# algbio/SBWT

Hardware: AMD Instinct MI355X
Metric: k-mers/sec (whole node), plain-matrix k=30 streaming search (higher is better)
Workload: dtype u64

## Files before the change

### sbwt_amd/csrc/sbwt_device.h

```cpp
#pragma once
#include <stdint.h>

#ifndef SBWT_MEGA_SHIFT
#define SBWT_MEGA_SHIFT 31
#endif
static_assert(SBWT_MEGA_SHIFT >= 7 && SBWT_MEGA_SHIFT <= 31, "a mega block holds 2 .. 2^25 whole 64-column blocks, and its relative counts fit 32 bits");
#define SBWT_GROUP_BASES 32

#ifndef SBWT_FUSED_SORT_DEFAULT
#define SBWT_FUSED_SORT_DEFAULT 3632
#endif
struct SbwtIndexView {
    const uint4 *blocks;
    const longlong2 *ptab;
    const unsigned long long *mega;
    long long n_nodes;
    long long n_pos;
    long long C[4];
    int k;
    int p_dev;
    int n_mega;
    int has_ssup;
    int probe_len;
    const uint4 *stab;
    int p_sparse;
    unsigned n_sb;
    const unsigned *col, *pos;
    const uint4 *pq;
    int has_safe;
    const uint4 *stab2;
    unsigned n_sb2;
    const uint4 *pfil;
    int p_filter, log2f;
    const uint4 *trans;
    unsigned n_tslots;
    int stab_pos;
    int debug;
    int out32 = 0;
    int big = 0;
    int fused_sort = 0;
    int force_mega;
};

struct SbwtBlobHeader {
    uint64_t magic;
    int64_t n_nodes, n_kmers, k, p_file, p_dev;
    int64_t C[4];
    int64_t n_blocks, n_mega;
    int64_t off_blocks, off_ptab, off_ftab, off_mega, blob_bytes;
    int32_t has_ssup;
    int32_t rank_only;
    int32_t ssup_derived;
    int32_t p_sparse;
    int64_t off_stab;
    int32_t big_layout;
    int32_t has_path;
    int64_t off_col, off_pos, off_pq, off_trans;
    int32_t stab_pos;
    int32_t p_filter;
    int64_t off_pfil;
    int32_t log2f;
    int32_t has_safe;
    int32_t force_mega;
    int64_t n_tslots;
    int64_t n_sb;
    int64_t n_pos;
    int64_t n_trans;
    int64_t n_paths;
    int64_t n_branch;
    int64_t image_level;
    int64_t row_ones[4];
    int32_t log2b2_unused;
    int64_t n_sb2;
    int64_t off_stab2;
    int64_t path_lookahead;
};
#define SBWT_BLOB_MAGIC 0x3355504754574253ull

#define SBWT_SP_EMPTY (1ull << 63)
#define SBWT_SP_OVERFLOW (1ull << 62)
#define SBWT_SP_UNIQ 0x80000000u
#define SBWT_SP_MAX_DEPTH 31
#define SBWT_SP_HASH 0x9E3779B97F4A7C15ull
static __host__ __device__ inline unsigned long long sp2_hash(unsigned origin, unsigned long long key2) {
    unsigned long long h = (key2 ^ ((unsigned long long)origin << 17)) * SBWT_SP_HASH;
    h ^= h >> 31;
    return (h + origin) * 0xD6E8FEB86659FD93ull;
}
#define SBWT_SP2_USED 0x80000000u
#define SBWT_SP2_OVERFLOW 0x80000000u
static __host__ __device__ inline unsigned long long sbwt_pf_hash(unsigned long long key) { return key * SBWT_SP_HASH; }
static __host__ __device__ inline unsigned sbwt_pf_bits(unsigned long long h) { return (unsigned)(h >> 24) ^ (unsigned)(h >> 41); }

struct SbwtWorkHeader {
    unsigned long long ticket;
    int status;
    int rg_sample;
    unsigned long long n_stream;
    unsigned long long n_search;
    unsigned long long n_lf;
    unsigned long long n_tab_hit;
    unsigned long long n_ext;
    unsigned long long n_bridge;
    unsigned long long u_bad;
    long long u_read0, u_len, u_out0, u_stride;
    unsigned long long n_deferred;
    unsigned long long ticket2;
    unsigned long long n_pieces;
    unsigned long long pad[15];
    unsigned long long rg_long;
    unsigned long long n_ftick;
    unsigned long long ftick_over;
    unsigned long long pad2[5];
    unsigned long long hint;
};
#define SBWT_WS_CLEAR_BYTES (sizeof(SbwtWorkHeader) - 8)

#define SBWT_PIECE 1024
struct SbwtPieceTab {
    uint4 *pairs = nullptr;
    uint4 *outs = nullptr;
    long long cap = 0;
    int piece = SBWT_PIECE;
};
static_assert(sizeof(SbwtWorkHeader) == 320, "workspace header is 320 bytes");
struct SbwtTickTab {
    uint4 *tick = nullptr;
    unsigned *tick_read = nullptr;
    unsigned *defer_bits = nullptr;
    long long cap = 0;
};
#define SBWT_HINT_MAGIC 0x5B377A00u
#define SBWT_HINT_RATIO 12
#define SBWT_HINT_CALLS 2

void sbwt_launch_encode(const char *d_bases, long long total_bases, uint4 *d_packed, SbwtWorkHeader *ws,
                        hipStream_t stream);
void sbwt_launch_search(const SbwtIndexView &ix, const uint4 *d_packed, const long long *d_read_off,
                        const long long *d_out_off, long long *d_out, long long n_reads, SbwtWorkHeader *ws,
                        int streaming, hipStream_t stream, int variant, long long total_groups, void *d_sort_scratch,
                        long long sort_scratch_bytes, int sort_key_bits, SbwtPieceTab pt);
void sbwt_launch_search_fused(const SbwtIndexView &ix, const char *d_bases, long long total_bases, uint4 *d_packed,
                              const long long *d_read_off, const long long *d_out_off, long long *d_out, long long n_reads,
                              SbwtWorkHeader *ws, int streaming, hipStream_t stream, unsigned *d_defer,
                              hipEvent_t ev_begin, hipEvent_t ev_end, SbwtPieceTab pt, int ragged_ok, SbwtTickTab tt = SbwtTickTab());
void sbwt_launch_encode_chained(const char *d_bases, long long total_bases, uint4 *d_packed, SbwtWorkHeader *ws,
                                const unsigned *d_defer, const long long *d_read_off, int k, hipStream_t stream);
void sbwt_launch_search_chained(const SbwtIndexView &ix, const uint4 *d_packed, const long long *d_read_off,
                                const long long *d_out_off, long long *d_out, long long n_reads, SbwtWorkHeader *ws,
                                int streaming, hipStream_t stream, const unsigned *d_defer, SbwtPieceTab pt);
void sbwt_launch_piece_bounds_tt(const uint4 *d_packed, const long long *d_read_off, const long long *d_out_off, int k,
                                 SbwtWorkHeader *ws, SbwtPieceTab pt, int behind_fused, hipStream_t stream, const unsigned *defer_bits);
void sbwt_launch_piece_bounds(const uint4 *d_packed, const long long *d_read_off, const long long *d_out_off, int k,
                              SbwtWorkHeader *ws, SbwtPieceTab pt, int behind_fused, hipStream_t stream);
long long sbwt_sort_scratch_bytes(long long n_reads, int key_bits);
const unsigned *sbwt_launch_sort_reads(const SbwtIndexView &ix, const uint4 *d_packed, const long long *d_read_off,
                                       long long n_reads, const SbwtWorkHeader *ws, void *d_scratch, long long scratch_bytes,
                                       int key_bits, hipStream_t stream);
void sbwt_launch_rank(const SbwtIndexView &ix, const long long *d_pos, const char *d_sym, long long n,
                      long long *d_out, hipStream_t stream);
void sbwt_launch_precalc(const SbwtIndexView &ix, int p, longlong2 *d_table, hipStream_t stream);
void sbwt_launch_update_interval(const SbwtIndexView &ix, const char *d_bases, const long long *d_off, long long n,
                                 long long *d_first, long long *d_second, hipStream_t stream);
void sbwt_launch_forward(const SbwtIndexView &ix, const long long *d_node, const char *d_sym, long long n,
                         long long *d_out, hipStream_t stream);
void sbwt_launch_partial_search(const SbwtIndexView &ix, const char *d_bases, const long long *d_off, long long n,
                                long long *d_first, long long *d_second, long long *d_matched, hipStream_t stream);
void sbwt_launch_get_kmer(const SbwtIndexView &ix, const long long *d_colex, long long n, char *d_out,
                          hipStream_t stream);
void sbwt_launch_select(const SbwtIndexView &ix, const long long *d_j, const char *d_sym, long long n,
                        const long long row_ones[4], long long *d_out, hipStream_t stream);
long long sbwt_format_scratch_bytes(long long n_reads);
void sbwt_launch_format(const long long *d_vals, const long long *d_out_off, long long n_reads, char *d_text,
                        long long *d_line_off, void *d_scratch, hipStream_t stream);
long long sbwt_blocks_scratch_bytes(long long n_nodes);
int sbwt_blocks_count(const unsigned long long *d_bits, long long n_nodes, void *d_scratch, long long totals[5], hipStream_t st);
void sbwt_blocks_fill(const unsigned long long *d_bits, const unsigned long long *d_ssup, long long n_nodes, void *d_scratch,
                      const long long C[4], int use_mega, int n_mega, uint4 *d_blocks, unsigned long long *d_mega, hipStream_t st);
long long sbwt_derive_scratch_bytes(long long n_nodes);
void sbwt_launch_derive_marks(const SbwtIndexView &ix, uint4 *d_blocks, void *d_scratch, hipStream_t stream);
long long sbwt_sparse_scratch_bytes(long long n_nodes);
long long sbwt_path_scratch_bytes(long long n_nodes);
long long sbwt_path_quads(long long n_nodes);
long long sbwt_count_paths(const SbwtIndexView &ix, hipStream_t stream);
void sbwt_launch_path_safe(const SbwtIndexView &ix, uint4 *d_pq, int rule, void *d_hlab, unsigned char *d_alt_safe,
                           hipStream_t stream);
long long sbwt_path_safe_scratch_bytes(long long n_pos, int k);
long long sbwt_launch_path_oth(const SbwtIndexView &ix, uint4 *d_pq, long long *n_branch, hipStream_t stream, int count_only = 0);
void sbwt_launch_trans_insert(const SbwtIndexView &ix, uint4 *d_trans, long long n_slots, const unsigned char *d_alt_safe,
                              hipStream_t stream);
int sbwt_launch_build_path(const SbwtIndexView &ix, unsigned *d_col, unsigned *d_pos, uint4 *d_pq, long long pos_cap,
                           long long *n_pos, int stitch, int min_copy, void *d_scratch, int lookahead, hipStream_t stream);
int sbwt_launch_build_sparse(const SbwtIndexView &ix, int p_dense, int p_sparse, long long n_buckets, uint4 *d_table,
                             void *d_scratch, const unsigned *d_pos, int p_filter, int log2f, uint4 *d_filter,
                             long long n_entries2, uint4 *d_table2, hipStream_t stream);

struct SbwtBuildState {
    int k = 0, rc = 0, ssup = 0;
    int key_bytes = 8;
    long long n_text = 0, nk = 0, ng = 0, n_nopred = 0;
    void *km = nullptr;
    unsigned *edges = nullptr;
    void *nopred_keys = nullptr;
};
int sbwt_build_phase_a(const char *h_text, long long n_text, int k, int rc, SbwtBuildState *S, hipStream_t st);
int sbwt_build_from_keys(void *d_km, long long nk, int k, SbwtBuildState *S, hipStream_t st);
int sbwt_build_copy_nopred(const SbwtBuildState *S, void *h_keys);
int sbwt_build_phase_b(SbwtBuildState *S, const void *h_ddata, const unsigned *h_dedges, long long nd, int ssup,
                       unsigned long long *h_rows, hipStream_t st);
void sbwt_build_release(SbwtBuildState *S);
```

### sbwt_amd/csrc/sbwt_search_fused.hip

```cpp
#include "sbwt_kernels_common.h"

#define F_IDLE 0
#define F_INIT 2
#define F_STEP 3
#define F_DEAD 4
#define F_EXT 7
#define F_TRANS 8
#define F_POS 9
#define F_BRIDGE 10
#define F_CMP 11
#define F_PLAN 12
#define FE_NONE 0
#define FE_EMIT1 1
#define FE_FAIL 2
#define FE_END 3
#define FE_PRES 4
#define FE_ANCH 5
#ifndef FZ_ANCHORS
#define FZ_ANCHORS 3
#endif
#ifndef FZ_ALIGNS
#define FZ_ALIGNS 7
#endif
#define CF_S1 1u
#define CF_A1 2u
#define CF_B1 4u
#define CF_S2 8u
#define CF_A2 16u
#define CF_B2 32u
#define CF_ONP 64u
#define CF_ALIGNED 128u
#define CF_ANCH 256u
#define CF_SEED 512u
#define CA_GOON 0
#define CA_DONE 1
#define CA_CERT 2
#define CA_TRANS 3
#define CA_ABSENT 4
#define CA_LOST 5
#define CF_MISS 1024u
#define CF_MISS_MASK 3072u
#define CF_WIN31 8192u
#define CF_SEED2 16384u
#define CF_NOCERT 4096u
#define CF_FORCE (1u << 30)
#define CF_ANC_LEFT(f) (((f) >> 16) & 3u)
#define CF_CMP_LEFT(f) (((f) >> 18) & 7u)
#define CF_ANC_TRIED(f) ((int)(((f) >> 21) & 511u) - 1)
#define CF_SET_TRIED(f, a) ((f) = ((f) & ~(511u << 21)) | ((((unsigned)((a) + 1)) & 511u) << 21))
#define CF_BUDGETS (((unsigned)FZ_ANCHORS << 16) | ((unsigned)FZ_ALIGNS << 18))
#define CF_M1 (CF_S1 | CF_A1 | CF_B1)
#define CF_M2 (CF_S2 | CF_A2 | CF_B2)

#ifndef FZ_SPLIT_MIN
#define FZ_SPLIT_MIN 16
#endif
#define FZ_NSEG 9

typedef unsigned fz_u32x4 __attribute__((ext_vector_type(4)));

#ifdef SBWT_STATS
#ifndef SBWT_SLOW_LO
#define SBWT_SLOW_LO 100
#define SBWT_SLOW_HI 100000
#endif
__device__ unsigned long long g_iter_hist[64];
__device__ unsigned long long g_tail_prof[192];
extern "C" int sbwtgpu_debug_tail_prof(unsigned long long *out, int reset) {
    if (out && hipMemcpyFromSymbol(out, HIP_SYMBOL(g_tail_prof), sizeof(g_tail_prof)) != hipSuccess) return -1;
    if (reset) {
        unsigned long long z[192] = {0};
        if (hipMemcpyToSymbol(HIP_SYMBOL(g_tail_prof), z, sizeof(z)) != hipSuccess) return -1;
    }
    return 0;
}
__device__ unsigned long long g_iter_max[8];
extern "C" int sbwtgpu_debug_iter_hist(unsigned long long *out, int reset) {
    if (out && hipMemcpyFromSymbol(out, HIP_SYMBOL(g_iter_hist), sizeof(g_iter_hist)) != hipSuccess) return -1;
    if (reset) {
        unsigned long long z[64] = {0};
        if (hipMemcpyToSymbol(HIP_SYMBOL(g_iter_hist), z, sizeof(z)) != hipSuccess) return -1;
    }
    return 0;
}
extern "C" int sbwtgpu_debug_iter_max(unsigned long long *out, int reset) {
    if (out && hipMemcpyFromSymbol(out, HIP_SYMBOL(g_iter_max), sizeof(g_iter_max)) != hipSuccess) return -1;
    if (reset) {
        unsigned long long z[8] = {0};
        if (hipMemcpyToSymbol(HIP_SYMBOL(g_iter_max), z, sizeof(z)) != hipSuccess) return -1;
    }
    return 0;
}
__device__ unsigned long long g_fz_why[24];
extern "C" int sbwtgpu_debug_why(unsigned long long *out, int reset) {
    if (out && hipMemcpyFromSymbol(out, HIP_SYMBOL(g_fz_why), sizeof(g_fz_why)) != hipSuccess) return -1;
    if (reset) {
        unsigned long long z[24] = {0};
        if (hipMemcpyToSymbol(HIP_SYMBOL(g_fz_why), z, sizeof(z)) != hipSuccess) return -1;
    }
    return 0;
}
__device__ unsigned long long g_sort_stats[16];
extern "C" int sbwtgpu_debug_sort_stats(unsigned long long *out, int reset) {
    if (out && hipMemcpyFromSymbol(out, HIP_SYMBOL(g_sort_stats), sizeof(g_sort_stats)) != hipSuccess) return -1;
    if (reset) {
        unsigned long long z[16] = {0};
        if (hipMemcpyToSymbol(HIP_SYMBOL(g_sort_stats), z, sizeof(z)) != hipSuccess) return -1;
    }
    return 0;
}
#define FZ_SORT_STAT(q, val) do { const unsigned long long v_ = (unsigned long long)(val); if (lane == 0 && v_) atomicAdd(&g_sort_stats[q], v_); } while (0)
#define FZ_WHY(q, cond) do { const unsigned long long n_ = __popcll(__ballot(cond)); if (lane == 0 && n_) atomicAdd(&g_fz_why[q], n_); } while (0)
__device__ unsigned long long g_fz_plan[48];
extern "C" int sbwtgpu_debug_plan(unsigned long long *out, int reset) {
    if (out && hipMemcpyFromSymbol(out, HIP_SYMBOL(g_fz_plan), sizeof(g_fz_plan)) != hipSuccess) return -1;
    if (reset) {
        unsigned long long z[48] = {0};
        if (hipMemcpyToSymbol(HIP_SYMBOL(g_fz_plan), z, sizeof(z)) != hipSuccess) return -1;
    }
    return 0;
}
#define FZ_PLAN(q, cond) do { const unsigned long long n_ = __popcll(__ballot(cond)); if (lane == 0 && n_) atomicAdd(&g_fz_plan[q], n_); } while (0)
#define FZ_PLAN_SUM(q, val) do { unsigned long long v_ = (unsigned long long)(val); for (int o_ = 32; o_ > 0; o_ >>= 1) v_ += __shfl_down(v_, o_); if (lane == 0 && v_) atomicAdd(&g_fz_plan[q], v_); } while (0)
#define FZ_HIST_FLUSH() do { if (it_cnt) { atomicAdd(&g_iter_hist[(it_cnt >> 1) < 63 ? (it_cnt >> 1) : 63], 1ull); \
    if (it_cnt >= SBWT_SLOW_LO && it_cnt < SBWT_SLOW_HI) atomicMax(&g_iter_max[it_cnt & 7u], ((unsigned long long)it_cnt << 32) | rd); it_cnt = 0; } } while (0)
#else
#define FZ_SORT_STAT(q, val) do { } while (0)
#define FZ_HIST_FLUSH() do { } while (0)
#define FZ_WHY(q, cond) do { } while (0)
#define FZ_PLAN(q, cond) do { } while (0)
#define FZ_PLAN_SUM(q, val) do { } while (0)
#endif

#ifdef SBWT_TIMELINE
__device__ unsigned long long g_fz_tl[8];
__device__ unsigned long long g_fz_tl_hist[1024];
extern "C" int sbwtgpu_debug_timeline(unsigned long long *out, int reset) {
    if (out && (hipMemcpyFromSymbol(out, HIP_SYMBOL(g_fz_tl), sizeof(g_fz_tl)) != hipSuccess ||
                hipMemcpyFromSymbol(out + 8, HIP_SYMBOL(g_fz_tl_hist), sizeof(g_fz_tl_hist)) != hipSuccess)) return -1;
    if (reset) {
        static unsigned long long z[1024];
        unsigned long long t0[8] = {~0ull, ~0ull, 0, 0, 0, 0, 0, 0};
        if (hipMemcpyToSymbol(HIP_SYMBOL(g_fz_tl), t0, sizeof(t0)) != hipSuccess ||
            hipMemcpyToSymbol(HIP_SYMBOL(g_fz_tl_hist), z, sizeof(g_fz_tl_hist)) != hipSuccess) return -1;
    }
    return 0;
}
#endif

__device__ __forceinline__ u64 fz_encode32(const unsigned w[8], const unsigned tm[8], unsigned &bad) {
    u64 codes = 0;
#pragma unroll
    for (int d = 0; d < 8; d++) {
        const unsigned x = w[d];
        const unsigned t = ((x >> 1) & 0x03030303u) ^ ((x >> 2) & 0x01010101u);
        const unsigned c8 = (t * 0x01041040u) >> 24;
        const unsigned letters = __builtin_amdgcn_perm(0x54474341u, 0x54474341u, t);
        bad |= (letters ^ x) & tm[d];
        codes |= (u64)c8 << (8 * d);
    }
    return codes;
}

#ifdef FZ_SORT_WG5
#define FZ_SLOTS 256
#define FZ_RING 256
#define FZ_SORT_WGS 5
#else
#define FZ_SLOTS 320
#define FZ_RING 512
#define FZ_SORT_WGS 4
#endif
template <bool WIDE, bool O32, bool BIG = false, bool UNI = false, bool SORT = false, bool TAB = false>
__global__ void __launch_bounds__(256, SORT ? FZ_SORT_WGS : 5) k_search_fused(SbwtIndexView ix, const unsigned char *__restrict__ bases,
                                                          i64 total_bases, i64 *__restrict__ out, i64 n_reads,
                                                          SbwtWorkHeader *ws, unsigned *__restrict__ defer_list,
                                                          const i64 *__restrict__ read_off, const i64 *__restrict__ out_off,
                                                          SbwtTickTab tt) {
    static_assert(!SORT || (!WIDE && !BIG), "lanes sorted by state: k <= 31, fewer than 2^31 columns (so far)");
    __shared__ u64 pool_codes[SBWT_FUSED_MAXG][SORT ? 128 : 256];
    constexpr int NSLOT = SORT ? FZ_SLOTS : 256;
    __shared__ u64 cur_codes[SBWT_FUSED_MAXG][NSLOT];
    __shared__ unsigned seg_src[FZ_NSEG][NSLOT];
    __shared__ unsigned char seg_at[FZ_NSEG][NSLOT];
    __shared__ unsigned st_w[SORT ? 4 : 1][SORT ? FZ_SLOTS : 1];
    __shared__ unsigned short q_ring[SORT ? 2 : 1][SORT ? FZ_RING : 1];
    __shared__ unsigned q_ctl[8];
    const int fmode = sbwt_fused_mode(ws, ix.k);
    if (fmode == 0) return;
    const int P_batch = sbwt_fused_pieces(ws, ix.k);
    if (UNI != (fmode == 1 && P_batch == 1 && !(ix.debug & 128))) return;
    const bool ragged = !UNI && fmode == 2;
    static_assert(!TAB || !UNI, "the ticket table's instantiation is a general one");
    const bool table = TAB && fmode == 3 && tt.tick != nullptr;
    if (TAB != (fmode == 3)) return;
    if (!WIDE && !BIG && ix.fused_sort > 0) {
        const bool sorted_call = (ix.fused_sort & 4096) ||
                                 (ws->hint == (unsigned long long)(SBWT_HINT_MAGIC | (unsigned)SBWT_HINT_CALLS) && (UNI || TAB || P_batch == 1));
        if (SORT != sorted_call) return;
    } else if (SORT) return;
    const int tid = threadIdx.x, lane = tid & 63, wbase = tid & ~63;
    const bool follower_wave = SORT && __builtin_amdgcn_readfirstlane(tid) >= 128;
    int slot = SORT ? (follower_wave ? -1 : tid) : tid;
    if (SORT) {
        if (tid < 8) q_ctl[tid] = (tid == 2) ? (unsigned)(FZ_SLOTS - 128) : 0u;
        for (int q = tid; q < (SORT ? FZ_RING : 0); q += 256) {
            q_ring[0][SORT ? q : 0] = q < FZ_SLOTS - 128 ? (unsigned short)(128 + q + 1) : (unsigned short)0;
            q_ring[SORT ? 1 : 0][SORT ? q : 0] = 0;
        }
        for (int q = 128 + tid; q < (SORT ? FZ_SLOTS : 0); q += 256) st_w[SORT ? 2 : 0][SORT ? q : 0] = 0u;
        __syncthreads();
    }
#define FZ_LDS32(p) (*(__attribute__((address_space(3))) volatile unsigned *)(p))
#define FZ_LDS16(p) (*(__attribute__((address_space(3))) volatile unsigned short *)(p))
    auto ring_push = [&](const u64 mask, const int ring, const int s) {
        unsigned base = 0;
        if (lane == 0) base = __hip_atomic_fetch_add(&q_ctl[2 + ring], (unsigned)__popcll(mask), __ATOMIC_RELAXED, __HIP_MEMORY_SCOPE_WORKGROUP);
        base = uniform32(base);
        if ((mask >> lane) & 1ull) {
            const unsigned at = (base + (unsigned)__popcll(mask & low_mask(lane))) & (unsigned)(FZ_RING - 1);
            asm volatile("s_waitcnt lgkmcnt(0)" ::: "memory");
            FZ_LDS16(&q_ring[SORT ? ring : 0][SORT ? at : 0]) = (unsigned short)(s + 1);
        }
    };
    const int k = ix.k, p = ix.p_dev, L0 = ix.probe_len, ps = ix.p_sparse;
    const int P = (UNI || table) ? 1 : P_batch, kpp = SBWT_FUSED_MAXLEN - k + 1;
    const bool varlen = ragged || table || P > 1;
    const i64 n_tickets = table ? (i64)ws->n_ftick : n_reads * P;
    const int ulen = (ragged || table) ? SBWT_FUSED_MAXLEN : (int)ws->u_len, m = ulen - k + 1, G = varlen ? SBWT_FUSED_MAXG : ((ulen + 31) >> 5);
    const i64 u_read0 = ws->u_read0, u_out0 = ws->u_out0, u_stride = ws->u_stride;
    const bool pfon = ix.pfil && ix.p_filter == L0 && L0 > p;
    const u64 mk2 = (k - ps >= 32) ? ~0ull : low_mask(2 * ((k - ps) & 31));
    const int pw = pfon ? L0 : p;
    const int last_node = (int)(ix.n_nodes - 1);
    static_assert(!BIG || !O32, "2^31 columns and more: int64 results");
    auto zx = [](int v) -> i64 { return BIG ? (i64)(unsigned)v : (i64)v; };
    auto is_run = [](unsigned src) -> bool { return BIG ? src != 0xFFFFFFFFu : !(src >> 31); };

    int nseg = 0, i0 = 0, last_start = 0;
    unsigned sort_spins = 0;
    unsigned sort_seen = 0;
    unsigned sort_waits = 0;
#ifdef SBWT_SORT_COUNTERS
    unsigned c_iter = 0;
    unsigned long long c_busy = 0;
    unsigned c_lists = 0, c_part = 0;
#endif
    const int sort_thr = (SORT && (ix.fused_sort & 255) > 1) ? ((ix.fused_sort & 255) < 64 ? (ix.fused_sort & 255) : 64) : 0;
    const int sort_ship = SORT ? ((ix.fused_sort >> 8) & 15) : 0;
    u64 fm_pend = 0;
    int pend = 0;
    unsigned pend_rd = 0;
    unsigned last_src = 0, emit_pos = 0;
    int wk = 0;
    u64 hk = 0;
    int blo = -1;
    int co = 0, cP = 0, m1 = -1;
    unsigned fl = 0;
    const bool wide_k = WIDE && ((ix.stab2 != nullptr && ps < k) || (ix.stab_pos && ps == k)) && !(ix.debug & 32);
    const bool anch_ok = wide_k;
    const bool seed_ok = wide_k && ps < k && !BIG;
    int bnext = -1;
    int mode = F_IDLE;
    unsigned rd = 0;
    int i = 0, j = 0, b = -1, wstart = 0;
    int mend = 0;
    bool drained = false;
    int l = 0, r = 0;
    unsigned c_ext = 0;
    constexpr bool LSEG_LDS = SORT || !UNI;
    u64 pool_next = 0, pool_end = 0, pool_bad = 0;
    int pool_len = 0;
    unsigned c_stream = 0, c_search = 0, c_lf = 0, c_tab = 0;
#ifdef SBWT_STATS
    unsigned it_cnt = 0, tail_it = 0;
#endif
#ifdef SBWT_TIMELINE
    const u64 tl_start = wall_clock64();
    u64 tl_drain = 0;
    unsigned tl_n = 0;
    if (lane == 0) atomicMin(&g_fz_tl[0], tl_start);
#endif

    if (SORT && follower_wave) {
        constexpr bool isP = true;
        constexpr bool runS = !SORT || !isP, runP = !SORT || isP;
        constexpr int qc = isP ? 1 : 0;
#include "sbwt_search_fused_loop.inc"
    } else {
        constexpr bool isP = false;
        constexpr bool runS = !SORT || !isP, runP = !SORT || isP;
        constexpr int qc = isP ? 1 : 0;
#include "sbwt_search_fused_loop.inc"
    }

    FZ_HIST_FLUSH();
#ifdef SBWT_TIMELINE
    if (lane == 0) {
        const u64 tl_exit = wall_clock64(), t0 = g_fz_tl[0];
        atomicMin(&g_fz_tl[1], tl_drain); atomicMax(&g_fz_tl[2], tl_drain); atomicMax(&g_fz_tl[3], tl_exit);
        atomicAdd(&g_fz_tl[4], 1ull); atomicAdd(&g_fz_tl[5], tl_exit - tl_drain); atomicAdd(&g_fz_tl[6], tl_exit - tl_start);
        atomicAdd(&g_fz_tl[7], (unsigned long long)tl_n);
        const u64 bk = (tl_exit - t0) / 1000ull;
        atomicAdd(&g_fz_tl_hist[bk < 1023 ? bk : 1023], 1ull);
    }
#endif
    {
        u64 e = c_ext & 0xFFFFFu, eb = c_ext >> 20;
#pragma unroll
        for (int off = 32; off > 0; off >>= 1) { e += __shfl_down(e, off); eb += __shfl_down(eb, off); }
        if (lane == 0) { if (e) atomicAdd(&ws->n_ext, e); if (eb) atomicAdd(&ws->n_bridge, eb); }
    }
#if defined(SBWT_SORT_COUNTERS) && !defined(SBWT_STATS)
    if (SORT && lane == 0) {
        atomicAdd(&ws->pad[follower_wave ? 13 : 11], (unsigned long long)c_iter);
        atomicAdd(&ws->pad[follower_wave ? 14 : 12], c_busy);
        atomicAdd(&ws->pad[9], (unsigned long long)c_lists);
        atomicAdd(&ws->pad[10], (unsigned long long)c_part);
    }
#endif
    if (lane == 0) {
        if (c_stream) atomicAdd(&ws->n_stream, (u64)c_stream);
        if (c_search) atomicAdd(&ws->n_search, (u64)c_search);
        if (c_lf) atomicAdd(&ws->n_lf, (u64)c_lf);
        if (c_tab) atomicAdd(&ws->n_tab_hit, (u64)c_tab);
    }
}

__global__ void __launch_bounds__(256) k_fused_tickets(const i64 *__restrict__ read_off, const i64 *__restrict__ out_off, i64 n_reads,
                                                       SbwtWorkHeader *ws, int k, SbwtTickTab tt) {
    if (!sbwt_fused_wants_table(ws, k)) return;
    const int lane = threadIdx.x & 63;
    const int kpp = SBWT_FUSED_MAXLEN - k + 1;
    const i64 stride = (i64)gridDim.x * 256;
    for (i64 r0 = (i64)blockIdx.x * 256 + (threadIdx.x & ~63); r0 < n_reads; r0 += stride) {
        const i64 r = r0 + lane;
        const bool valid = r < n_reads;
        const i64 P0 = valid ? read_off[r] : 0, len = valid ? read_off[r + 1] - P0 : 0, ob = valid ? out_off[r] : 0;
        const i64 m = len - k + 1;
        const u64 np = m > 0 ? (u64)((m + kpp - 1) / kpp) : 0ull;
        u64 incl = np;
#pragma unroll
        for (int o = 1; o < 64; o <<= 1) { const u64 v = __shfl_up(incl, o); if (lane >= o) incl += v; }
        const u64 total = __shfl(incl, 63);
        if (total == 0) continue;
        u64 base = 0;
        if (lane == 0) base = atomicAdd(&ws->n_ftick, (unsigned long long)total);
        base = uniform64(base);
        if (base + total > (u64)tt.cap) {
            if (lane == 0) ws->ftick_over = 1ull;
            continue;
        }
        const u64 first = base + incl - np;
        auto entry = [&](i64 rr, i64 p0, i64 ln, i64 o0, u64 t0, u64 j) {
            const i64 b = p0 + (i64)j * kpp, left = ln - (i64)j * kpp;
            const unsigned nb = (unsigned)(left > SBWT_FUSED_MAXLEN ? SBWT_FUSED_MAXLEN : left);
            const i64 o = o0 + (i64)j * kpp;
            tt.tick[t0 + j] = make_uint4((unsigned)b, ((unsigned)((u64)b >> 32) & 0xFFFFu) | (nb << 16), (unsigned)o, (unsigned)((u64)o >> 32));
            tt.tick_read[t0 + j] = (unsigned)rr;
        };
        for (u64 j = 0; j < np && j < 4; j++) entry(r, P0, len, ob, first, j);
        u64 big = __ballot(np > 4);
        while (big) {
            const int src = __ffsll((i64)big) - 1;
            big &= big - 1;
            const i64 rr = __shfl(r, src), p0 = __shfl(P0, src), ln = __shfl(len, src), o0 = __shfl(ob, src);
            const u64 t0 = __shfl(first, src), nn = __shfl(np, src);
            for (u64 j = 4 + (u64)lane; j < nn; j += 64) entry(rr, p0, ln, o0, t0, j);
        }
    }
}

__global__ void k_fused_hint(SbwtWorkHeader *ws, int k) {
    if (threadIdx.x != 0 || sbwt_fused_mode(ws, k) == 0) return;
    const unsigned long long ext = ws->n_ext, walks = ws->n_search, prev = ws->hint;
    const bool fits = walks > 0 && ext >= (unsigned long long)SBWT_HINT_RATIO * walks;
    const unsigned run = ((prev & ~0xFFull) == (unsigned long long)SBWT_HINT_MAGIC) ? (unsigned)(prev & 0xFFull) : 0u;
    ws->hint = (unsigned long long)(SBWT_HINT_MAGIC | (fits ? (run < SBWT_HINT_CALLS ? run + 1u : (unsigned)SBWT_HINT_CALLS) : 0u));
}

__global__ void __launch_bounds__(256) k_check_uniform2(const i64 *__restrict__ read_off, const i64 *__restrict__ out_off,
                                                        i64 n_reads, SbwtWorkHeader *ws, int k, SbwtPieceTab pt,
                                                        int rg_enable) {
    const i64 t = (i64)blockIdx.x * 256 + threadIdx.x;
    const i64 len = read_off[1] - read_off[0], stride = (n_reads > 1) ? out_off[1] - out_off[0] : 0;
    if (t == 0) { ws->u_read0 = read_off[0]; ws->u_len = len; ws->u_out0 = out_off[0]; ws->u_stride = stride; }
    const bool valid = t < n_reads;
    const i64 mylen = valid ? read_off[t + 1] - read_off[t] : 0;
    fused_sample_of_wave(t, mylen, valid, n_reads, rg_enable, k, ws);
    piece_zones_of_wave(t, mylen, valid, k, ws, pt);
    if (!valid) return;
    const bool bad = (mylen != len) || (t + 1 < n_reads && out_off[t + 1] - out_off[t] != stride);
    if (__ballot(bad) != 0 && (threadIdx.x & 63) == 0) ws->u_bad = 1ull;
}

void sbwt_launch_search_fused(const SbwtIndexView &ix, const char *d_bases, long long total_bases, uint4 *d_packed,
                              const long long *d_read_off, const long long *d_out_off, long long *d_out, long long n_reads,
                              SbwtWorkHeader *ws, int streaming, hipStream_t stream, unsigned *d_defer,
                              hipEvent_t ev_begin, hipEvent_t ev_end, SbwtPieceTab pt, int ragged_ok, SbwtTickTab tt) {
    if (n_reads <= 0) return;
    hipLaunchKernelGGL(k_check_uniform2, dim3(grid_for(n_reads)), dim3(256), 0, stream, d_read_off, d_out_off, (i64)n_reads, ws,
                       ix.k, pt, ragged_ok);
    if (tt.tick && n_reads < ((i64)1 << 32)) {
        const i64 wantt = (n_reads + 255) / 256;
        hipLaunchKernelGGL(k_fused_tickets, dim3((unsigned)(wantt < 1024 ? wantt : 1024)), dim3(256), 0, stream, d_read_off, d_out_off,
                           (i64)n_reads, ws, ix.k, tt);
    }
    const i64 want_r = (n_reads + 255) / 256, want_t = tt.tick ? (total_bases / SBWT_FUSED_MAXLEN + 255) / 256 : 0;
    const i64 want = want_r > want_t ? want_r : want_t;
    unsigned cap = 1280u;
    if (ix.debug >> 8) cap = (unsigned)(ix.debug >> 8);
    else if (total_bases < 8000000ll) cap = 256u;
    else if (total_bases < 20000000ll) cap = 384u;
    else if (total_bases < 60000000ll) cap = 512u;
    else if (total_bases < 110000000ll) cap = 640u;
    else if (total_bases < 170000000ll) cap = 768u;
    else if (total_bases < 250000000ll) cap = 896u;
    else if (total_bases < 500000000ll) cap = 1024u;
    const bool sorted = !ix.big && !(ix.n_nodes >= ((i64)1 << 31) - 64) && !((ix.stab2 != nullptr && ix.p_sparse < ix.k) || (ix.debug & 64)) && ix.fused_sort > 0;
    const unsigned cap_s = cap > 256u * FZ_SORT_WGS ? 256u * FZ_SORT_WGS : cap;
    const unsigned g = (unsigned)(want < (i64)cap ? want : (i64)cap), g_s = (unsigned)(want < (i64)cap_s ? want : (i64)cap_s);
    if (ev_begin) (void)hipEventRecord(ev_begin, stream);
    const bool wide = (ix.stab2 != nullptr && ix.p_sparse < ix.k) || (ix.debug & 64);
#define FZ_LAUNCH1(W, O, B, U) hipLaunchKernelGGL((k_search_fused<W, O, B, U>), dim3(g), dim3(256), 0, stream, ix, \
                                           reinterpret_cast<const unsigned char *>(d_bases), (i64)total_bases, d_out, (i64)n_reads, ws, d_defer, \
                                           d_read_off, d_out_off, tt)
#define FZ_LAUNCH(W, O, B) do { FZ_LAUNCH1(W, O, B, true); FZ_LAUNCH1(W, O, B, false); \
                                if (tt.tick) hipLaunchKernelGGL((k_search_fused<W, O, B, false, false, true>), dim3(g), dim3(256), 0, stream, ix, \
                                           reinterpret_cast<const unsigned char *>(d_bases), (i64)total_bases, d_out, (i64)n_reads, ws, d_defer, \
                                           d_read_off, d_out_off, tt); } while (0)
#define FZ_LAUNCH_S(O) do { hipLaunchKernelGGL((k_search_fused<false, O, false, true, true>), dim3(g_s), dim3(256), 0, stream, ix, \
                                           reinterpret_cast<const unsigned char *>(d_bases), (i64)total_bases, d_out, (i64)n_reads, ws, d_defer, \
                                           d_read_off, d_out_off, tt); \
                            hipLaunchKernelGGL((k_search_fused<false, O, false, false, true>), dim3(g_s), dim3(256), 0, stream, ix, \
                                           reinterpret_cast<const unsigned char *>(d_bases), (i64)total_bases, d_out, (i64)n_reads, ws, d_defer, \
                                           d_read_off, d_out_off, tt); \
                            if (tt.tick) hipLaunchKernelGGL((k_search_fused<false, O, false, false, true, true>), dim3(g_s), dim3(256), 0, stream, ix, \
                                           reinterpret_cast<const unsigned char *>(d_bases), (i64)total_bases, d_out, (i64)n_reads, ws, d_defer, \
                                           d_read_off, d_out_off, tt); } while (0)
    const bool big = ix.big || ix.n_nodes >= ((i64)1 << 31) - 64;
    if (big) { if (wide) FZ_LAUNCH(true, false, true); else FZ_LAUNCH(false, false, true); }
    else if (wide) { if (ix.out32) FZ_LAUNCH(true, true, false); else FZ_LAUNCH(true, false, false); }
    else {
        if (ix.out32) FZ_LAUNCH(false, true, false); else FZ_LAUNCH(false, false, false);
        if (sorted) { if (ix.out32) FZ_LAUNCH_S(true); else FZ_LAUNCH_S(false); }
    }
#undef FZ_LAUNCH_S
#undef FZ_LAUNCH
#undef FZ_LAUNCH1
    if (ev_end) (void)hipEventRecord(ev_end, stream);
    if (sorted) hipLaunchKernelGGL(k_fused_hint, dim3(1), dim3(64), 0, stream, ws, ix.k);
    sbwt_launch_encode_chained(d_bases, total_bases, d_packed, ws, d_defer, d_read_off, ix.k, stream);
    sbwt_launch_piece_bounds_tt(d_packed, d_read_off, d_out_off, ix.k, ws, pt, 1, stream, tt.defer_bits);
    sbwt_launch_search_chained(ix, d_packed, d_read_off, d_out_off, d_out, n_reads, ws, streaming, stream, d_defer, pt);
}
```

Before: 266.6 billion.

## Merge UNI/general fused kernel instantiations and fold hint update into last wave

Splits the fused search kernel into a device body plus a dispatcher template that can host several bodies, so the unsorted path launches one kernel covering the uniform and general modes instead of two. It drops the separate single-thread hint kernel: the last wave to finish, found through an atomic done counter, computes the hint and sets a taken flag that makes later hinted instantiations exit early. This cuts kernel launches and early-exit launch overhead per call. The cost is a per-wave atomic with a memory wait at kernel end and larger kernel code, which may raise register pressure.

```diff
diff --git a/sbwt_amd/csrc/sbwt_device.h b/sbwt_amd/csrc/sbwt_device.h
--- a/sbwt_amd/csrc/sbwt_device.h
+++ b/sbwt_amd/csrc/sbwt_device.h
@@ -111,7 +111,9 @@
     unsigned long long rg_long;
     unsigned long long n_ftick;
     unsigned long long ftick_over;
-    unsigned long long pad2[5];
+    unsigned long long fz_done;
+    unsigned long long fz_taken;
+    unsigned long long pad2[3];
     unsigned long long hint;
 };
 #define SBWT_WS_CLEAR_BYTES (sizeof(SbwtWorkHeader) - 8)
diff --git a/sbwt_amd/csrc/sbwt_search_fused.hip b/sbwt_amd/csrc/sbwt_search_fused.hip
--- a/sbwt_amd/csrc/sbwt_search_fused.hip
+++ b/sbwt_amd/csrc/sbwt_search_fused.hip
@@ -171,34 +171,23 @@
 #define FZ_RING 512
 #define FZ_SORT_WGS 4
 #endif
-template <bool WIDE, bool O32, bool BIG = false, bool UNI = false, bool SORT = false, bool TAB = false>
-__global__ void __launch_bounds__(256, SORT ? FZ_SORT_WGS : 5) k_search_fused(SbwtIndexView ix, const unsigned char *__restrict__ bases,
-                                                          i64 total_bases, i64 *__restrict__ out, i64 n_reads,
-                                                          SbwtWorkHeader *ws, unsigned *__restrict__ defer_list,
-                                                          const i64 *__restrict__ read_off, const i64 *__restrict__ out_off,
-                                                          SbwtTickTab tt) {
+template <bool WIDE, bool O32, bool BIG, bool UNI, bool SORT, bool TAB>
+__device__ __forceinline__ void fz_search_body(const SbwtIndexView &ix, const unsigned char *__restrict__ bases,
+                                               i64 total_bases, i64 *__restrict__ out, i64 n_reads,
+                                               SbwtWorkHeader *ws, unsigned *__restrict__ defer_list,
+                                               const i64 *__restrict__ read_off, const i64 *__restrict__ out_off,
+                                               const SbwtTickTab &tt, const int fmode, const int P_batch,
+                                               u64 (&pool_codes)[SBWT_FUSED_MAXG][SORT ? 128 : 256],
+                                               u64 (&cur_codes)[SBWT_FUSED_MAXG][SORT ? FZ_SLOTS : 256],
+                                               unsigned (&seg_src)[FZ_NSEG][SORT ? FZ_SLOTS : 256],
+                                               unsigned char (&seg_at)[FZ_NSEG][SORT ? FZ_SLOTS : 256],
+                                               unsigned (&st_w)[SORT ? 4 : 1][SORT ? FZ_SLOTS : 1],
+                                               unsigned short (&q_ring)[SORT ? 2 : 1][SORT ? FZ_RING : 1],
+                                               unsigned (&q_ctl)[8]) {
     static_assert(!SORT || (!WIDE && !BIG), "lanes sorted by state: k <= 31, fewer than 2^31 columns (so far)");
-    __shared__ u64 pool_codes[SBWT_FUSED_MAXG][SORT ? 128 : 256];
-    constexpr int NSLOT = SORT ? FZ_SLOTS : 256;
-    __shared__ u64 cur_codes[SBWT_FUSED_MAXG][NSLOT];
-    __shared__ unsigned seg_src[FZ_NSEG][NSLOT];
-    __shared__ unsigned char seg_at[FZ_NSEG][NSLOT];
-    __shared__ unsigned st_w[SORT ? 4 : 1][SORT ? FZ_SLOTS : 1];
-    __shared__ unsigned short q_ring[SORT ? 2 : 1][SORT ? FZ_RING : 1];
-    __shared__ unsigned q_ctl[8];
-    const int fmode = sbwt_fused_mode(ws, ix.k);
-    if (fmode == 0) return;
-    const int P_batch = sbwt_fused_pieces(ws, ix.k);
-    if (UNI != (fmode == 1 && P_batch == 1 && !(ix.debug & 128))) return;
     const bool ragged = !UNI && fmode == 2;
     static_assert(!TAB || !UNI, "the ticket table's instantiation is a general one");
     const bool table = TAB && fmode == 3 && tt.tick != nullptr;
-    if (TAB != (fmode == 3)) return;
-    if (!WIDE && !BIG && ix.fused_sort > 0) {
-        const bool sorted_call = (ix.fused_sort & 4096) ||
-                                 (ws->hint == (unsigned long long)(SBWT_HINT_MAGIC | (unsigned)SBWT_HINT_CALLS) && (UNI || TAB || P_batch == 1));
-        if (SORT != sorted_call) return;
-    } else if (SORT) return;
     const int tid = threadIdx.x, lane = tid & 63, wbase = tid & ~63;
     const bool follower_wave = SORT && __builtin_amdgcn_readfirstlane(tid) >= 128;
     int slot = SORT ? (follower_wave ? -1 : tid) : tid;
@@ -324,6 +313,63 @@
         if (c_search) atomicAdd(&ws->n_search, (u64)c_search);
         if (c_lf) atomicAdd(&ws->n_lf, (u64)c_lf);
         if (c_tab) atomicAdd(&ws->n_tab_hit, (u64)c_tab);
+    }
+}
+
+__device__ __forceinline__ void fz_note_hint(SbwtWorkHeader *ws) {
+    const unsigned long long ext = __hip_atomic_load(&ws->n_ext, __ATOMIC_RELAXED, __HIP_MEMORY_SCOPE_AGENT),
+                             walks = __hip_atomic_load(&ws->n_search, __ATOMIC_RELAXED, __HIP_MEMORY_SCOPE_AGENT), prev = ws->hint;
+    const bool fits = walks > 0 && ext >= (unsigned long long)SBWT_HINT_RATIO * walks;
+    const unsigned run = ((prev & ~0xFFull) == (unsigned long long)SBWT_HINT_MAGIC) ? (unsigned)(prev & 0xFFull) : 0u;
+    ws->hint = (unsigned long long)(SBWT_HINT_MAGIC | (fits ? (run < SBWT_HINT_CALLS ? run + 1u : (unsigned)SBWT_HINT_CALLS) : 0u));
+}
+
+#define FZ_B_UNI 1
+#define FZ_B_GEN 2
+#define FZ_B_TAB 4
+#define FZ_B_ALL 7
+template <bool WIDE, bool O32, bool BIG, bool SORT, int BODIES>
+__global__ void __launch_bounds__(256, SORT ? FZ_SORT_WGS : 5) k_search_fused(SbwtIndexView ix, const unsigned char *__restrict__ bases,
+                                                          i64 total_bases, i64 *__restrict__ out, i64 n_reads,
+                                                          SbwtWorkHeader *ws, unsigned *__restrict__ defer_list,
+                                                          const i64 *__restrict__ read_off, const i64 *__restrict__ out_off,
+                                                          SbwtTickTab tt) {
+    __shared__ u64 pool_codes[SBWT_FUSED_MAXG][SORT ? 128 : 256];
+    constexpr int NSLOT = SORT ? FZ_SLOTS : 256;
+    __shared__ u64 cur_codes[SBWT_FUSED_MAXG][NSLOT];
+    __shared__ unsigned seg_src[FZ_NSEG][NSLOT];
+    __shared__ unsigned char seg_at[FZ_NSEG][NSLOT];
+    __shared__ unsigned st_w[SORT ? 4 : 1][SORT ? FZ_SLOTS : 1];
+    __shared__ unsigned short q_ring[SORT ? 2 : 1][SORT ? FZ_RING : 1];
+    __shared__ unsigned q_ctl[8];
+    const int fmode = sbwt_fused_mode(ws, ix.k);
+    if (fmode == 0) return;
+    const int P_batch = sbwt_fused_pieces(ws, ix.k);
+    const bool uni = fmode == 1 && P_batch == 1 && !(ix.debug & 128);
+    const bool tab = fmode == 3;
+    if (!(BODIES & (tab ? FZ_B_TAB : uni ? FZ_B_UNI : FZ_B_GEN))) return;
+    const bool hinted = !WIDE && !BIG && ix.fused_sort > 0;
+    if (hinted) {
+        const bool sorted_call = (ix.fused_sort & 4096) ||
+                                 (ws->hint == (unsigned long long)(SBWT_HINT_MAGIC | (unsigned)SBWT_HINT_CALLS) && (uni || tab || P_batch == 1));
+        if (SORT != sorted_call) return;
+        if (ws->fz_taken != 0) return;
+    } else if (SORT) return;
+#define FZ_BODY(U, T) fz_search_body<WIDE, O32, BIG, U, SORT, T>(ix, bases, total_bases, out, n_reads, ws, defer_list, read_off, out_off, tt, \
+                                                                 fmode, P_batch, pool_codes, cur_codes, seg_src, seg_at, st_w, q_ring, q_ctl)
+    if (tab) { if constexpr ((BODIES & FZ_B_TAB) != 0) FZ_BODY(false, true); }
+    else if (uni) { if constexpr ((BODIES & FZ_B_UNI) != 0) FZ_BODY(true, false); }
+    else { if constexpr ((BODIES & FZ_B_GEN) != 0) FZ_BODY(false, false); }
+#undef FZ_BODY
+    if (hinted && (threadIdx.x & 63) == 0) {
+        __builtin_amdgcn_fence(__ATOMIC_RELEASE, "workgroup");
+        asm volatile("s_waitcnt vmcnt(0)" ::: "memory");
+        const unsigned long long n_waves = (unsigned long long)gridDim.x * 4ull;
+        if (atomicAdd(&ws->fz_done, 1ull) + 1ull == n_waves) {
+            __threadfence();
+            fz_note_hint(ws);
+            ws->fz_taken = 1ull;
+        }
     }
 }
 
@@ -371,14 +417,6 @@
     }
 }
 
-__global__ void k_fused_hint(SbwtWorkHeader *ws, int k) {
-    if (threadIdx.x != 0 || sbwt_fused_mode(ws, k) == 0) return;
-    const unsigned long long ext = ws->n_ext, walks = ws->n_search, prev = ws->hint;
-    const bool fits = walks > 0 && ext >= (unsigned long long)SBWT_HINT_RATIO * walks;
-    const unsigned run = ((prev & ~0xFFull) == (unsigned long long)SBWT_HINT_MAGIC) ? (unsigned)(prev & 0xFFull) : 0u;
-    ws->hint = (unsigned long long)(SBWT_HINT_MAGIC | (fits ? (run < SBWT_HINT_CALLS ? run + 1u : (unsigned)SBWT_HINT_CALLS) : 0u));
-}
-
 __global__ void __launch_bounds__(256) k_check_uniform2(const i64 *__restrict__ read_off, const i64 *__restrict__ out_off,
                                                         i64 n_reads, SbwtWorkHeader *ws, int k, SbwtPieceTab pt,
                                                         int rg_enable) {
@@ -422,22 +460,17 @@
     const unsigned g = (unsigned)(want < (i64)cap ? want : (i64)cap), g_s = (unsigned)(want < (i64)cap_s ? want : (i64)cap_s);
     if (ev_begin) (void)hipEventRecord(ev_begin, stream);
     const bool wide = (ix.stab2 != nullptr && ix.p_sparse < ix.k) || (ix.debug & 64);
-#define FZ_LAUNCH1(W, O, B, U) hipLaunchKernelGGL((k_search_fused<W, O, B, U>), dim3(g), dim3(256), 0, stream, ix, \
+#define FZ_LAUNCH1(W, O, B, S, BODIES, G) hipLaunchKernelGGL((k_search_fused<W, O, B, S, BODIES>), dim3(G), dim3(256), 0, stream, ix, \
                                            reinterpret_cast<const unsigned char *>(d_bases), (i64)total_bases, d_out, (i64)n_reads, ws, d_defer, \
                                            d_read_off, d_out_off, tt)
-#define FZ_LAUNCH(W, O, B) do { FZ_LAUNCH1(W, O, B, true); FZ_LAUNCH1(W, O, B, false); \
-                                if (tt.tick) hipLaunchKernelGGL((k_search_fused<W, O, B, false, false, true>), dim3(g), dim3(256), 0, stream, ix, \
-                                           reinterpret_cast<const unsigned char *>(d_bases), (i64)total_bases, d_out, (i64)n_reads, ws, d_defer, \
-                                           d_read_off, d_out_off, tt); } while (0)
-#define FZ_LAUNCH_S(O) do { hipLaunchKernelGGL((k_search_fused<false, O, false, true, true>), dim3(g_s), dim3(256), 0, stream, ix, \
-                                           reinterpret_cast<const unsigned char *>(d_bases), (i64)total_bases, d_out, (i64)n_reads, ws, d_defer, \
-                                           d_read_off, d_out_off, tt); \
-                            hipLaunchKernelGGL((k_search_fused<false, O, false, false, true>), dim3(g_s), dim3(256), 0, stream, ix, \
-                                           reinterpret_cast<const unsigned char *>(d_bases), (i64)total_bases, d_out, (i64)n_reads, ws, d_defer, \
-                                           d_read_off, d_out_off, tt); \
-                            if (tt.tick) hipLaunchKernelGGL((k_search_fused<false, O, false, false, true, true>), dim3(g_s), dim3(256), 0, stream, ix, \
-                                           reinterpret_cast<const unsigned char *>(d_bases), (i64)total_bases, d_out, (i64)n_reads, ws, d_defer, \
-                                           d_read_off, d_out_off, tt); } while (0)
+#define FZ_LAUNCH(W, O, B) do { FZ_LAUNCH1(W, O, B, false, FZ_B_UNI | FZ_B_GEN, g); \
+                                if (tt.tick) FZ_LAUNCH1(W, O, B, false, FZ_B_TAB, g); } while (0)
+#ifdef FZ_SORT_MERGED
+#define FZ_LAUNCH_S(O) FZ_LAUNCH1(false, O, false, true, FZ_B_ALL, g_s)
+#else
+#define FZ_LAUNCH_S(O) do { FZ_LAUNCH1(false, O, false, true, FZ_B_UNI, g_s); FZ_LAUNCH1(false, O, false, true, FZ_B_GEN, g_s); \
+                            if (tt.tick) FZ_LAUNCH1(false, O, false, true, FZ_B_TAB, g_s); } while (0)
+#endif
     const bool big = ix.big || ix.n_nodes >= ((i64)1 << 31) - 64;
     if (big) { if (wide) FZ_LAUNCH(true, false, true); else FZ_LAUNCH(false, false, true); }
     else if (wide) { if (ix.out32) FZ_LAUNCH(true, true, false); else FZ_LAUNCH(true, false, false); }
@@ -449,7 +482,6 @@
 #undef FZ_LAUNCH
 #undef FZ_LAUNCH1
     if (ev_end) (void)hipEventRecord(ev_end, stream);
-    if (sorted) hipLaunchKernelGGL(k_fused_hint, dim3(1), dim3(64), 0, stream, ws, ix.k);
     sbwt_launch_encode_chained(d_bases, total_bases, d_packed, ws, d_defer, d_read_off, ix.k, stream);
     sbwt_launch_piece_bounds_tt(d_packed, d_read_off, d_out_off, ix.k, ws, pt, 1, stream, tt.defer_bits);
     sbwt_launch_search_chained(ix, d_packed, d_read_off, d_out_off, d_out, n_reads, ws, streaming, stream, d_defer, pt);
```

Result: no change. 266.9 billion, median of 6 (+0.1%).
